# cvxgrp/pymde

Measured on AMD Instinct MI355X. Metric: edges/sec/iter (avg_distortion fwd+bwd), n=1M |E|=50M d=2, higher is better.
Workload: dtype f32; 1 GPU; BASELINE configs[3] / SURVEY 8d config 4a: n=1000000, |E|=50000000 uniform-random edges (out-degree 50), d=2, penalties.Log1p(1.5), weights in {1,2}; seeded on the device with torch.Generator(0) (the survey's recipe uses numpy default_rng(0): same distribution, another stream; --survey-seed builds that one); parallelism=single GPU, parameter_stream=codebook: 2 distinct weights ride in the packed half-edge word (4 B/half-edge)

## Files before the change

### pymde_amd/csrc/mde_ring_kernel.h

```cpp
#pragma once
#include <algorithm>
#include <cstring>
#include <type_traits>
#include <vector>

#include "mde_ring.h"
#define COMMA ,

#define MDE_RING23(FN, LIN)                                    \
  do {                                                         \
    FN fn{a};                                                  \
    int rc;                                                    \
    if (A.d == 2)                                              \
      rc = launch_ring<2, FN, LIN>(A, fn, nblocks);            \
    else                                                       \
      rc = launch_ring<3, FN, LIN>(A, fn, nblocks);            \
    return rc == MDE_OK ? 1 : rc;                              \
  } while (0)

typedef uint32_t ring_u4 __attribute__((ext_vector_type(4)));
typedef float ring_f4 __attribute__((ext_vector_type(4)));

template <int D>
struct RingVec;
template <>
struct RingVec<1> {
  typedef float T;
};
template <>
struct RingVec<2> {
  typedef float2 T;
};
template <>
struct RingVec<4> {
// ... 41 lines not shown
    q[0] = v[0];
    q[1] = v[1];
    q[2] = v[2];
  } else {
    typename RingVec<D>::T t;
    float* q = reinterpret_cast<float*>(&t);
#pragma unroll
    for (int c = 0; c < D; ++c) q[c] = v[c];
    *reinterpret_cast<typename RingVec<D>::T*>(p) = t;
  }
}

__device__ __forceinline__ void ring_ctrl_store(uint32_t addr, int v) {
  asm volatile("ds_write_b32 %0, %1" ::"v"(addr), "v"(v) : "memory");
}
__device__ __forceinline__ void ring_ctrl_store_counted(char* lds_base, uint32_t addr, int v) {
  typedef __attribute__((address_space(3))) volatile int* lds_vint;
  *(lds_vint)(lds_base + addr) = v;
}
__device__ __forceinline__ int ring_ctrl_load(uint32_t addr) {
  int v;
  asm volatile("ds_read_b32 %0, %1\n\ts_waitcnt lgkmcnt(0)" : "=&v"(v) : "v"(addr) : "memory");
  return v;
}

#if MDE_RING_ABLATE
static __device__ unsigned long long g_ring_probe[8][1024];
static __device__ int g_ring_diag[64][8];
static __device__ int g_ring_ndiag;
#ifndef MDE_RING_SPINMAX
#define MDE_RING_SPINMAX 100000
#endif
#define RING_CLK() __builtin_readcyclecounter()
#endif
#ifndef MDE_RING_FWORDS
#define MDE_RING_FWORDS 0
#endif
#ifdef MDE_RING_EVAL2
constexpr bool defined_MDE_RING_EVAL2 = true;
#else
constexpr bool defined_MDE_RING_EVAL2 = false;
#endif
template <int D, class Fn, bool HAS_GRAD, int PS, bool LIN>
__global__ __launch_bounds__(MDE_RING_BS) void k_fused_ring(
    int nloc, int row_lo, int n, int R, int Q, int NC, int ring_off, int S, const int32_t* __restrict__ wave_iter,
    const uint32_t* __restrict__ hdr, const uint32_t* __restrict__ packed, const uint32_t* __restrict__ bidx,
    const int32_t* __restrict__ slot_row, const float* __restrict__ a0, const float* __restrict__ a1, int a0_scalar, int a1_scalar,
    const float* __restrict__ X,
    float* __restrict__ grad, float* __restrict__ partial, double* __restrict__ loss_partials, Fn fn,
    float fix_value, float grad_scale, float* __restrict__ loss_out, double loss_scale, int fold, int dbg_arg) {
#if MDE_RING_ABLATE
#ifndef MDE_RING_ABLATE_MASK
#define MDE_RING_ABLATE_MASK (~0)
#endif
  const int dbg = dbg_arg & (MDE_RING_ABLATE_MASK);
#else
  constexpr int dbg = 0;
#endif
  constexpr int BS = MDE_RING_BS, NCW = MDE_RING_NCW, NPROD = MDE_RING_NPROD;
  constexpr bool CB = PS == 1, BX = PS == 2;
  constexpr int GR_OFF = ring_gr_off(D), CTRL_PROG = MDE_RING_CTRL_PROG(D), CTRL_F = MDE_RING_CTRL_F(D), CTRL_CB = MDE_RING_CTRL_CB(D);
  constexpr int C = ring_chunk_cols(D), CBYTES = ring_chunk_bytes(D), PIECES = CBYTES / 1024;
  static_assert(GR_OFF + (ring_row_cap(D) + 32) * 4 * D <= 65536 + GR_OFF && GR_OFF < 65536 && CTRL_CB + 32 < 65536,
                "region bases must fit the 16-bit offset of the LDS instructions");
  static_assert(NPROD <= 8 && NCW <= 16, "control-word layout");
  __shared__ __attribute__((aligned(16))) char L[MDE_RING_LDS_BYTES];
  float* XR = reinterpret_cast<float*>(L);
  float* GR = reinterpret_cast<float*>(L + GR_OFF);
  const int tid = threadIdx.x, lane = tid & 63;
  const int wave = __builtin_amdgcn_readfirstlane(tid >> 6);
  const int rb = blockIdx.x / Q, qg = blockIdx.x % Q;
  const int j_lo = (int)(((int64_t)qg * NC + Q - 1) / Q), j_hi = (int)(((int64_t)(qg + 1) * NC + Q - 1) / Q);
  const int r0 = rb * R;
  const int nr = min(R, nloc - r0);
  const uint32_t dummy_row = (uint32_t)R * 4u * (uint32_t)D;
  const float a0s = (a0_scalar && PS == 0) ? a0[0] : 1.0f;
  const uint32_t tab_off = (uint32_t)ring_off + (uint32_t)S * (uint32_t)CBYTES;
  const float a1s = (a1 && a1_scalar) ? a1[0] : 0.0f;
  const bool a1_arr = a1 && !a1_scalar;
  {
    float4* z = reinterpret_cast<float4*>(L + GR_OFF);
    const int nz = ((R + 32) * 4 * D + 15) / 16;
    for (int i = tid; i < nz; i += BS) z[i] = make_float4(0.f, 0.f, 0.f, 0.f);
    const float* Xrow = X + (size_t)(row_lo + r0) * D;
    if (slot_row) {
      const int32_t* sr = slot_row + (size_t)rb * R;
      for (int sl = tid; sl < R; sl += BS) {
        const int r = sr[sl];
        float xv[D];
#pragma unroll
        for (int c = 0; c < D; ++c) xv[c] = r >= 0 ? X[(size_t)(row_lo + r) * D + c] : 0.0f;
#pragma unroll
        for (int c = 0; c < D; ++c) XR[sl * D + c] = xv[c];
      }
    } else if ((reinterpret_cast<uintptr_t>(Xrow) & 15) == 0) {
      const ring_f4* X4 = reinterpret_cast<const ring_f4*>(Xrow);
      ring_f4* XR4 = reinterpret_cast<ring_f4*>(L);
      const int n4 = (nr * D) >> 2;
      for (int i0 = 0; i0 < n4; i0 += 8 * BS) {
        ring_f4 t[8];
#pragma unroll
        for (int k = 0; k < 8; ++k) t[k] = X4[min(i0 + tid + k * BS, max(n4 - 1, 0))];
#pragma unroll
        for (int k = 0; k < 8; ++k)
          if (i0 + tid + k * BS < n4) XR4[i0 + tid + k * BS] = t[k];
      }
      for (int i = (n4 << 2) + tid; i < nr * D; i += BS) XR[i] = Xrow[i];
    } else {
      for (int i = tid; i < nr * D; i += BS) XR[i] = Xrow[i];
    }
    if (tid < 32 * D) XR[R * D + tid] = 0.0f;
    int* prog = reinterpret_cast<int*>(L + CTRL_PROG);
    int* F = reinterpret_cast<int*>(L + CTRL_F);
    if (tid < 16) prog[tid] = (tid < NCW) ? j_lo : MDE_RING_DONE;
#if MDE_RING_FWORDS
    static_assert(NPROD == 4 && MDE_RING_UNIT == 1, "MDE_RING_FWORDS: four producers, one chunk per step");
    if (tid >= 16 && tid < 16 + NPROD) F[tid - 16] = (j_lo + (tid - 16) < j_hi) ? j_lo + (tid - 16) : MDE_RING_DONE;
#else
    if (tid == 16) F[0] = j_lo;
#endif
    if (CB && tid >= 32 && tid < 32 + MDE_RING_CB_VALUES)
      reinterpret_cast<float*>(L + CTRL_CB)[tid - 32] = a0[tid - 32] * Fn::kParamScale;
    if (BX && tid >= 64 && tid < 64 + MDE_RING_BX_VALUES)
      reinterpret_cast<float*>(L + tab_off)[tid - 64] = a0[tid - 64] * Fn::kParamScale;
  }
  __syncthreads();
  float loss = 0.0f, loss2 = 0.0f;

  if (wave >= NCW) {
    if (MDE_RING_PRODPRIO) __builtin_amdgcn_s_setprio(MDE_RING_PRODPRIO);
    const int p = wave - NCW;
    const char* Xb = reinterpret_cast<const char*>(X);
    const size_t nbytes = (size_t)n * D * 4;
    const size_t last16 = nbytes - 16;
    constexpr int DEPTH = MDE_RING_DEPTH, UNIT = MDE_RING_UNIT;
    ring_f4 buf[DEPTH][UNIT * PIECES];
    auto ld16 = [&](ring_f4& dst, const ring_f4* src) __attribute__((always_inline)) {
#if MDE_RING_ASMLOAD
      asm volatile("global_load_dwordx4 %0, %1, off" : "=v"(dst) : "v"(src) : "memory");
#else
      dst = *src;
#endif
    };
    auto fetch = [&](int k, int j0u) __attribute__((always_inline)) {
#pragma unroll
      for (int c = 0; c < UNIT; ++c) {
        const int j = j0u + c;
        if (j < NC - 1) {
          const ring_f4* src = reinterpret_cast<const ring_f4*>(Xb + (size_t)j * CBYTES + (size_t)lane * 16);
#pragma unroll
          for (int i = 0; i < PIECES; ++i) ld16(buf[k][c * PIECES + i], src + i * 64);
        } else {
          const size_t off0 = (size_t)min(j, NC - 1) * CBYTES + (size_t)lane * 16;
#pragma unroll
          for (int i = 0; i < PIECES; ++i) {
            const size_t off = off0 + (size_t)i * 1024;
            ld16(buf[k][c * PIECES + i], reinterpret_cast<const ring_f4*>(Xb + (off < last16 ? off : last16)));
          }
        }
// ... 8 lines not shown
      else if constexpr (UNIT * PIECES == 3)
        asm volatile("s_waitcnt vmcnt(%3)" : "+v"(buf[k][0]), "+v"(buf[k][1]), "+v"(buf[k][2]) : "n"(NEWER) : "memory");
      else if constexpr (UNIT * PIECES == 2)
        asm volatile("s_waitcnt vmcnt(%2)" : "+v"(buf[k][0]), "+v"(buf[k][1]) : "n"(NEWER) : "memory");
      else if constexpr (UNIT * PIECES == 6)
        asm volatile("s_waitcnt vmcnt(%6)" : "+v"(buf[k][0]), "+v"(buf[k][1]), "+v"(buf[k][2]), "+v"(buf[k][3]), "+v"(buf[k][4]),
                     "+v"(buf[k][5]) : "n"(NEWER) : "memory");
      else
        asm volatile("s_waitcnt vmcnt(%8)" : "+v"(buf[k][0]), "+v"(buf[k][1]), "+v"(buf[k][2]), "+v"(buf[k][3]), "+v"(buf[k][4]),
                     "+v"(buf[k][5]), "+v"(buf[k][6]), "+v"(buf[k][7]) : "n"(NEWER) : "memory");
#endif
    };
    ring_f4 tail_v = {0.0f, 0.0f, 0.0f, 0.0f};
    int tail_rel = -1;
    if ((nbytes & 15) != 0 && j_hi == NC) {
      const size_t off_str = nbytes & ~(size_t)15;
      const size_t rel = off_str - (size_t)(NC - 1) * CBYTES;
      if (off_str >= (size_t)(NC - 1) * CBYTES && lane == (int)((rel & 1023) >> 4)) {
        tail_rel = (int)rel;
        const float* tp = reinterpret_cast<const float*>(Xb + off_str);
        const int nt = (int)((nbytes - off_str) >> 2);
        tail_v[0] = tp[0];
        if (nt > 1) tail_v[1] = tp[1];
        if (nt > 2) tail_v[2] = tp[2];
      }
    }
    int minprog = j_lo, landed = j_lo;
    const uint32_t poll_addr = lane < 16 ? CTRL_PROG + 4u * (uint32_t)lane : (uint32_t)CTRL_F;
#if MDE_RING_ABLATE
    unsigned long long pr_t0 = RING_CLK(), pr_blocked = 0, pr_polls = 0, pr_chain = 0, pr_data = 0, pr_write = 0;
#endif
#pragma unroll
    for (int k = 0; k < DEPTH; ++k) fetch(k, j_lo + UNIT * (p + k * NPROD));
    int slot = (j_lo + UNIT * p) % S;
    for (int j0 = j_lo + UNIT * p; j0 < j_hi && !(dbg & 128); j0 += UNIT * DEPTH * NPROD) {
#pragma unroll
      for (int k = 0; k < DEPTH; ++k) {
        const int j = j0 + k * UNIT * NPROD;
        if (j < j_hi) {
          const int jl = min(j + UNIT, j_hi) - 1;
          while (jl - S >= minprog && !(dbg & 8)) {
#if MDE_RING_ABLATE
            const unsigned long long tb0 = RING_CLK();
            ++pr_polls;
#endif
            int v = ring_ctrl_load(poll_addr);
            asm volatile("s_nop 1\n\tv_min_i32_dpp %0, %0, %0 row_shr:1 row_mask:0xf bank_mask:0xf\n\t"
                         "s_nop 1\n\tv_min_i32_dpp %0, %0, %0 row_shr:2 row_mask:0xf bank_mask:0xf\n\t"
                         "s_nop 1\n\tv_min_i32_dpp %0, %0, %0 row_shr:4 row_mask:0xf bank_mask:0xf\n\ts_nop 1"
                         : "+v"(v));
            if (NCW > 8) asm volatile("v_min_i32_dpp %0, %0, %0 row_shr:8 row_mask:0xf bank_mask:0xf\n\ts_nop 1" : "+v"(v));
            minprog = __builtin_amdgcn_readlane(v, NCW <= 8 ? 7 : 15);
            landed = __builtin_amdgcn_readlane(v, 16);
            if (jl - S >= minprog) __builtin_amdgcn_s_sleep(MDE_RING_PSLEEP);
#if MDE_RING_ABLATE
            pr_blocked += RING_CLK() - tb0;
            if (pr_polls > MDE_RING_SPINMAX) {
              if (lane == 0) {
                const int kk = atomicAdd(&g_ring_ndiag, 1);
                if (kk < 64) {
                  int* r = g_ring_diag[kk];
                  r[0] = 2; r[1] = blockIdx.x; r[2] = p; r[3] = j; r[4] = minprog; r[5] = S; r[6] = j_lo; r[7] = j_hi;
                }
              }
              pr_polls = 0;
              minprog = jl;
// ... 15 lines not shown
            const int jc = j + c;
            if (UNIT > 1 && jc >= j_hi) break;
            int sc = slot + c;
            if (UNIT > 1 && sc >= S) sc -= S;
            char* dst = L + (uint32_t)__builtin_amdgcn_readfirstlane(ring_off + sc * CBYTES) + lane * 16;
#pragma unroll
            for (int i = 0; i < PIECES; ++i) *reinterpret_cast<ring_f4*>(dst + i * 1024) = buf[k][c * PIECES + i];
            if (jc == NC - 1 && tail_rel >= 0) *reinterpret_cast<ring_f4*>(dst - lane * 16 + tail_rel) = tail_v;
          }
          asm volatile("" ::: "memory");
#if MDE_RING_FWORDS
          (void)landed;
          ring_ctrl_store_counted(L, CTRL_F + 4u * (uint32_t)p, (j + NPROD < j_hi) ? j + NPROD : MDE_RING_DONE);
#else
          while (landed != j && !(dbg & 8)) {
            landed = __builtin_amdgcn_readfirstlane(ring_ctrl_load((uint32_t)CTRL_F + 0u * (uint32_t)lane));
#if MDE_RING_ABLATE
            ++pr_chain;
#endif
            if (landed != j) __builtin_amdgcn_s_sleep(0);
          }
          ring_ctrl_store_counted(L, CTRL_F, jl + 1);
#endif
#if MDE_RING_ABLATE
          if (dbg & 512) pr_write += RING_CLK() - td0;
#endif
          fetch(k, j + UNIT * DEPTH * NPROD);
          slot += UNIT * NPROD;
          while (slot >= S) slot -= S;
        }
      }
    }
#if MDE_RING_ABLATE
    if ((dbg & 512) && lane == 0 && blockIdx.x < 1024) {
      atomicAdd(&g_ring_probe[3][blockIdx.x], RING_CLK() - pr_t0);
      atomicAdd(&g_ring_probe[4][blockIdx.x], pr_blocked);
      atomicAdd(&g_ring_probe[6][blockIdx.x], pr_polls);
      atomicAdd(&g_ring_probe[5][blockIdx.x], pr_data);
      atomicAdd(&g_ring_probe[7][blockIdx.x], pr_write);
    }
#endif
  } else {
    if (MDE_RING_CONSPRIO) __builtin_amdgcn_s_setprio(MDE_RING_CONSPRIO);
    const int ib = __builtin_amdgcn_readfirstlane(wave_iter[blockIdx.x * NCW + wave]);
    const int NB = (__builtin_amdgcn_readfirstlane(wave_iter[blockIdx.x * NCW + wave + 1]) - ib) >> 2;
    if (NB > 0 && !(dbg & 64)) {
      const bool a0_arr = !a0_scalar && PS == 0;
      const uint32_t* bp = BX ? bidx + (size_t)(ib >> 2) * 64 + lane : nullptr;
      const ring_u4* sp = reinterpret_cast<const ring_u4*>(packed) + (size_t)(ib >> 2) * 64 + lane;
      const ring_f4* ap = reinterpret_cast<const ring_f4*>(a0_arr ? a0 : reinterpret_cast<const float*>(packed)) +
                          (size_t)(ib >> 2) * 64 + lane;
      const int lastb = NB - 1;
      constexpr int PFB = MDE_RING_PFB;
      ring_u4 pq[PFB] = {};
      uint32_t hv[PFB] = {};
      ring_f4 wq[PFB] = {};
      uint32_t bq[PFB] = {};
      const uint32_t* hvp = hdr + (size_t)ib * MDE_RING_HW + (lane & 15);
      auto load_block = [&](int u, int b) __attribute__((always_inline)) {
        const int bc = min(b, lastb);
#if defined(MDE_RING_STREAM_L2)
        pq[u] = sp[(size_t)(bc & 7) * 64];
#elif defined(MDE_RING_STREAM_NT)
        pq[u] = __builtin_nontemporal_load(&sp[(size_t)bc * 64]);
#else
        pq[u] = sp[(size_t)bc * 64];
#endif
        hv[u] = hvp[(size_t)bc * 16];
        if (PS == 0) wq[u] = ap[(size_t)bc * 64];
        if (BX) bq[u] = bp[(size_t)bc * 64];
      };
#if MDE_RING_ABLATE
      unsigned long long cs_t0 = RING_CLK(), cs_poll = 0, cs_trips = 0;
#endif

      struct Pre {
        float xr[D], xc[D], p0;
#ifdef MDE_RING_KEEPROW
        uint32_t row;
#endif
      };
#ifdef MDE_RING_PROBE_ROWLIN
      auto row_of = [&](uint32_t w) __attribute__((always_inline)) { return ((w & 0x7f00u) | ((uint32_t)lane << 3)) & 0xfff8u; };
#else
      auto row_of = [&](uint32_t w) __attribute__((always_inline)) { return D == 2 ? (w & 0xfff8u) : (w & 0xfffcu); };
#endif
#ifdef MDE_RING_PROBE_COLLIN
      auto col_of = [&](uint32_t w) __attribute__((always_inline)) {
        return (((w >> 13) & 0x3f000u) | ((uint32_t)lane << 3)) & 0x3fff8u;
      };
#else
      auto col_of = [&](uint32_t w) __attribute__((always_inline)) {
        return D == 2 ? ((w >> 13) & 0x3fff8u) : ((w >> 14) & 0x3fffcu);
      };
#endif
      auto issue_x = [&](uint32_t w, float p0, uint32_t bi4) __attribute__((always_inline)) {
        Pre r;
        if constexpr (BX)
          r.p0 = *reinterpret_cast<const float*>(L + tab_off + bi4);
        else
          r.p0 = CB ? *reinterpret_cast<const float*>(L + CTRL_CB + ((w & (D == 2 ? 7u : 3u)) << 2)) : p0 * Fn::kParamScale;
#ifdef MDE_RING_KEEPROW
        r.row = row_of(w);
        ring_ld_operand<D>(L, r.row, r.xr);
// ... 136 lines not shown

      Pre xa, xb;
      float acc[D], accb[D];
      auto block_body = [&](auto lc_tag, int u, int b) __attribute__((always_inline)) {
#pragma unroll
        for (int h = 0; h < 2; ++h) {
          const int q = 2 * h;
          const int un = h == 0 ? u : (u + 1) % PFB, qn = (q + 2) & 3;
          wait_pair(un, qn);
          const Pre xna = issue_x(pq[un][qn], (a0_scalar || PS != 0) ? a0s : wq[un][qn], bx4(bq[un], qn));
          const Pre xnb = issue_x(pq[un][qn + 1], (a0_scalar || PS != 0) ? a0s : wq[un][qn + 1], bx4(bq[un], qn + 1));
          release_to((u + 1) % PFB, q);
          prefetch_landed();
          const float p1a = a1_arr ? a1[((size_t)((ib >> 2) + b) * 64 + lane) * 4 + q] : a1s;
          const float p1b = a1_arr ? a1[((size_t)((ib >> 2) + b) * 64 + lane) * 4 + q + 1] : a1s;
          const bool lc2 = decltype(lc_tag)::value == 2;
          const uint32_t hma = lc2 ? (uint32_t)__builtin_amdgcn_readlane((int)hv[u], 4 * q) : 0u;
          const uint32_t hmb = lc2 ? (uint32_t)__builtin_amdgcn_readlane((int)hv[u], 4 * q + 4) : 0u;
          finish(lc_tag, pq[u][q], xa, acc, p1a, hma);
          if (HAS_GRAD) {
            const bool same = row_of(pq[u][q + 1]) == row_of(pq[u][q]);
#pragma unroll
            for (int c = 0; c < D; ++c) accb[c] = same ? acc[c] : accb[c];
          }
          finish(lc_tag, pq[u][q + 1], xb, accb, p1b, hmb);
          if (HAS_GRAD) {
            ring_ld<D>(L + GR_OFF + row_of(pq[un][qn]), acc);
            ring_ld<D>(L + GR_OFF + row_of(pq[un][qn + 1]), accb);
          }
          xa = xna;
          xb = xnb;
        }
      };
#pragma unroll
      for (int u = 0; u < PFB; ++u) load_block(u, u);
      release_to(0, 0);
      wait_pair(0, 0);
      xa = issue_x(pq[0][0], (a0_scalar || PS != 0) ? a0s : wq[0][0], bx4(bq[0], 0));
      xb = issue_x(pq[0][1], (a0_scalar || PS != 0) ? a0s : wq[0][1], bx4(bq[0], 1));
      release_to(0, 2);
      prefetch_landed();
      if (HAS_GRAD) {
        ring_ld<D>(L + GR_OFF + row_of(pq[0][0]), acc);
        ring_ld<D>(L + GR_OFF + row_of(pq[0][1]), accb);
      }
      for (int base = 0; base < NB; base += PFB) {
#pragma unroll
        for (int u = 0; u < PFB; ++u) {
          const int b = base + u;
          if (b < NB) {
            const int bcls = __builtin_amdgcn_readlane((int)hv[u], 3) & 3;
            if (bcls == 0)
              block_body(std::integral_constant<int, 0>(), u, b);
            else if (bcls == 1)
              block_body(std::integral_constant<int, 1>(), u, b);
            else
              block_body(std::integral_constant<int, 2>(), u, b);
          }
          load_block(u, b + PFB);
        }
      }
#if MDE_RING_ABLATE
      if ((dbg & 512) && lane == 0 && blockIdx.x < 1024) {
        atomicAdd(&g_ring_probe[0][blockIdx.x], RING_CLK() - cs_t0);
        atomicAdd(&g_ring_probe[1][blockIdx.x], cs_poll);
        atomicAdd(&g_ring_probe[2][blockIdx.x], cs_trips);
      }
#endif
    }
    if constexpr (Fn::kRingFused) loss = fmaf(loss, 0.6931471805599453f, loss2) * (1.0f / Fn::kParamScale);
    ring_ctrl_store_counted(L, CTRL_PROG + 4u * (uint32_t)wave, MDE_RING_DONE);
    __builtin_amdgcn_s_waitcnt(0x0F70);
  }
  __syncthreads();
  if (HAS_GRAD && slot_row) {
    const int32_t* sr = slot_row + (size_t)rb * R;
    if (fold) {
      unsigned int* sync = reinterpret_cast<unsigned int*>(partial + (size_t)Q * nloc * D) + 2 * rb;
      int* tk = reinterpret_cast<int*>(L + 512);
      if (tid == 0) *tk = (int)__hip_atomic_fetch_add(&sync[0], 1u, __ATOMIC_RELAXED, __HIP_MEMORY_SCOPE_AGENT);
      __syncthreads();
      const bool second = *tk != 0;
      float* mine = partial + (size_t)qg * nloc * D;
      const float* other = partial + (size_t)(1 - qg) * nloc * D;
      if (!second) {
        for (int sl = tid; sl < R; sl += BS) {
          const int r = sr[sl];
          if (r < 0) continue;
#pragma unroll
          for (int c = 0; c < D; ++c)
            __hip_atomic_store(mine + (size_t)r * D + c, GR[sl * D + c], __ATOMIC_RELAXED, __HIP_MEMORY_SCOPE_AGENT);
        }
        __builtin_amdgcn_s_waitcnt(0x0F70);
        __syncthreads();
        if (tid == 0) __hip_atomic_store(&sync[1], 1u, __ATOMIC_RELAXED, __HIP_MEMORY_SCOPE_AGENT);
      } else {
        if (tid == 0) {
          while (__hip_atomic_load(&sync[1], __ATOMIC_RELAXED, __HIP_MEMORY_SCOPE_AGENT) == 0u) __builtin_amdgcn_s_sleep(2);
          __hip_atomic_store(&sync[1], 0u, __ATOMIC_RELAXED, __HIP_MEMORY_SCOPE_AGENT);
          __hip_atomic_store(&sync[0], 0u, __ATOMIC_RELAXED, __HIP_MEMORY_SCOPE_AGENT);
        }
        __syncthreads();
        for (int s0 = 0; s0 < R; s0 += 8 * BS) {
          int rr[8];
          float o[8][D];
#pragma unroll
          for (int k = 0; k < 8; ++k) rr[k] = s0 + tid + k * BS < R ? sr[s0 + tid + k * BS] : -1;
#pragma unroll
          for (int k = 0; k < 8; ++k)
#pragma unroll
            for (int c = 0; c < D; ++c)
              o[k][c] = __hip_atomic_load(other + (size_t)max(rr[k], 0) * D + c, __ATOMIC_RELAXED, __HIP_MEMORY_SCOPE_AGENT);
#pragma unroll
          for (int k = 0; k < 8; ++k) {
            if (rr[k] < 0) continue;
            const int sl = s0 + tid + k * BS;
#pragma unroll
            for (int c = 0; c < D; ++c) {
              const float m = GR[sl * D + c];
              grad[(size_t)(row_lo + rr[k]) * D + c] = (qg == 0 ? m + o[k][c] : o[k][c] + m) * grad_scale;
            }
          }
        }
      }
      __syncthreads();
    } else {
      float* dst = (Q == 1) ? grad + (size_t)row_lo * D : partial + (size_t)qg * nloc * D;
      const float sc = (Q == 1) ? grad_scale : 1.0f;
      for (int sl = tid; sl < R; sl += BS) {
        const int r = sr[sl];
        if (r < 0) continue;
#pragma unroll
        for (int c = 0; c < D; ++c) dst[(size_t)r * D + c] = GR[sl * D + c] * sc;
      }
    }
  } else if (HAS_GRAD && fold) {
    unsigned int* sync = reinterpret_cast<unsigned int*>(partial + (size_t)Q * nloc * D) + 2 * rb;
    int* tk = reinterpret_cast<int*>(L + 512);
    if (tid == 0) *tk = (int)__hip_atomic_fetch_add(&sync[0], 1u, __ATOMIC_RELAXED, __HIP_MEMORY_SCOPE_AGENT);
    __syncthreads();
    const bool second = *tk != 0;
    float* mine = partial + ((size_t)qg * nloc + r0) * D;
    const float* other = partial + ((size_t)(1 - qg) * nloc + r0) * D;
    float* grow = grad + (size_t)(row_lo + r0) * D;
    static_assert(GR_OFF % 16 == 0, "16-byte accumulator pieces");
    const bool vec = ((reinterpret_cast<uintptr_t>(mine) | reinterpret_cast<uintptr_t>(other) | reinterpret_cast<uintptr_t>(grow)) & 15) == 0;
    const int n4 = vec ? (nr * D) >> 2 : 0, n1 = nr * D;
    const ring_f4* GR4 = reinterpret_cast<const ring_f4*>(GR);
    if (!second) {
      for (int i = tid; i < n4; i += BS) {
        const ring_f4 v4 = GR4[i];
        asm volatile("global_store_dwordx4 %0, %1, off sc1" ::"v"(reinterpret_cast<ring_f4*>(mine) + i), "v"(v4) : "memory");
      }
      for (int i = (n4 << 2) + tid; i < n1; i += BS) __hip_atomic_store(mine + i, GR[i], __ATOMIC_RELAXED, __HIP_MEMORY_SCOPE_AGENT);
      __builtin_amdgcn_s_waitcnt(0x0F70);
      __syncthreads();
      if (tid == 0) __hip_atomic_store(&sync[1], 1u, __ATOMIC_RELAXED, __HIP_MEMORY_SCOPE_AGENT);
    } else {
      if (tid == 0) {
        while (__hip_atomic_load(&sync[1], __ATOMIC_RELAXED, __HIP_MEMORY_SCOPE_AGENT) == 0u) __builtin_amdgcn_s_sleep(2);
        __hip_atomic_store(&sync[1], 0u, __ATOMIC_RELAXED, __HIP_MEMORY_SCOPE_AGENT);
        __hip_atomic_store(&sync[0], 0u, __ATOMIC_RELAXED, __HIP_MEMORY_SCOPE_AGENT);
      }
      __syncthreads();
      const ring_f4* o4p = reinterpret_cast<const ring_f4*>(other);
      for (int i0 = 0; i0 < n4; i0 += 8 * BS) {
        ring_f4 o[8];
#pragma unroll
        for (int k = 0; k < 8; ++k)
          asm volatile("global_load_dwordx4 %0, %1, off sc1" : "=v"(o[k]) : "v"(o4p + min(i0 + tid + k * BS, n4 - 1)) : "memory");
        asm volatile("s_waitcnt vmcnt(0)" : "+v"(o[0]), "+v"(o[1]), "+v"(o[2]), "+v"(o[3]), "+v"(o[4]), "+v"(o[5]), "+v"(o[6]), "+v"(o[7])::"memory");
#pragma unroll
        for (int k = 0; k < 8; ++k) {
          const int i = i0 + tid + k * BS;
          if (i < n4) {
            const ring_f4 m = GR4[i];
            reinterpret_cast<ring_f4*>(grow)[i] = (qg == 0 ? m + o[k] : o[k] + m) * grad_scale;
          }
        }
      }
      for (int i0 = n4 << 2; i0 < n1; i0 += 8 * BS) {
        float o[8];
#pragma unroll
        for (int k = 0; k < 8; ++k) o[k] = __hip_atomic_load(other + min(i0 + tid + k * BS, n1 - 1), __ATOMIC_RELAXED, __HIP_MEMORY_SCOPE_AGENT);
#pragma unroll
        for (int k = 0; k < 8; ++k) {
          const int i = i0 + tid + k * BS;
          if (i < n1) grow[i] = (qg == 0 ? GR[i] + o[k] : o[k] + GR[i]) * grad_scale;
        }
      }
    }
    __syncthreads();
  } else if (HAS_GRAD) {
    float* grow = (Q == 1) ? grad + (size_t)(row_lo + r0) * D : partial + ((size_t)qg * nloc + r0) * D;
    const float sc = (Q == 1) ? grad_scale : 1.0f;
    const int n4 = (reinterpret_cast<uintptr_t>(grow) & 15) == 0 ? (nr * D) >> 2 : 0;
    for (int i = tid; i < n4; i += BS) reinterpret_cast<ring_f4*>(grow)[i] = reinterpret_cast<const ring_f4*>(GR)[i] * sc;
    for (int i = (n4 << 2) + tid; i < nr * D; i += BS) grow[i] = GR[i] * sc;
  }
  double* red = reinterpret_cast<double*>(L);
  unsigned int* ticket = reinterpret_cast<unsigned int*>(loss_partials + MDE_MAX_PARTIALS);
  const double v = mde_wave_sum((double)loss);
  if (lane == 0) red[wave] = v;
  __syncthreads();
  if (tid == 0) {
    double s = 0.0;
    for (int i = 0; i < NCW; ++i) s += red[i];
    mde_st_partial(loss_partials + blockIdx.x, s);
  }
  int* last_flag = reinterpret_cast<int*>(L + 256);
  __builtin_amdgcn_s_waitcnt(0x0F70);
  __syncthreads();
  if (tid == 0) {
    const unsigned int k = __hip_atomic_fetch_add(ticket, 1u, __ATOMIC_RELAXED, __HIP_MEMORY_SCOPE_AGENT);
    *last_flag = (k == gridDim.x - 1u) ? 1 : 0;
    if (*last_flag) __hip_atomic_store(ticket, 0u, __ATOMIC_RELAXED, __HIP_MEMORY_SCOPE_AGENT);
  }
  __syncthreads();
  if (!*last_flag) return;
  double t = 0.0;
  for (int i = tid; i < (int)gridDim.x; i += BS) t += mde_ld_partial(loss_partials + i);
  t = mde_wave_sum(t);
  __syncthreads();
  if (lane == 0) red[wave] = t;
  __syncthreads();
  if (tid == 0) {
    double s = 0.0;
    for (int i = 0; i < BS / 64; ++i) s += red[i];
    *loss_out = (float)(s * loss_scale);
    loss_partials[MDE_PARTIALS_LOSS_D] = s * loss_scale;
  }
}

template <class V>
__global__ __launch_bounds__(MDE_BLOCK) void k_ring_combine(int64_t m, int Q, const V* __restrict__ partial,
                                                            float scale, V* __restrict__ out) {
  constexpr int W = sizeof(V) / sizeof(float);
  const int64_t i = (int64_t)blockIdx.x * MDE_BLOCK + threadIdx.x;
  if (i >= m) return;
  V a[8];
#pragma unroll
  for (int q = 0; q < 8; ++q)
    if (q < Q) a[q] = partial[(size_t)q * m + i];
  float s[W];
#pragma unroll
  for (int k = 0; k < W; ++k) s[k] = reinterpret_cast<const float*>(&a[0])[k];
#pragma unroll
  for (int q = 1; q < 8; ++q)
    if (q < Q) {
#pragma unroll
      for (int k = 0; k < W; ++k) s[k] += reinterpret_cast<const float*>(&a[q])[k];
// ... 38 lines not shown
  const uint32_t* bidx = bx ? reinterpret_cast<const uint32_t*>(A.a0) : nullptr;
  const float* a0 = cb ? A.a0 + L.H : (bx ? A.a0 + L.H / 4 : A.a0);
  const int Q = L.col_groups;
  *nblocks = L.n_row_blocks * Q;
  const float out_scale = A.grad_scale * A.inv_p;
  const float fix_value = A.inv_p > 0.0f ? 1.0f / A.inv_p : 1.0f;
#if MDE_RING_ABLATE
  const int dbg = getenv("MDE_RING_DBG") ? atoi(getenv("MDE_RING_DBG")) : 0;
#else
  const int dbg = 0;
#endif
  static const int fold_env = getenv("MDE_RING_FOLD") ? atoi(getenv("MDE_RING_FOLD")) : 1;
  const int fold = (Q == 2 && A.grad && fold_env) ? 1 : 0;
  hipLaunchKernelGGL(kern, dim3(L.n_row_blocks * Q), dim3(MDE_RING_BS), 0, A.st,
                     (int)(A.plan->row_hi - A.plan->row_lo), (int)A.plan->row_lo, (int)A.plan->n,
                     L.rows_per_block, Q, L.n_chunks, L.ring_off, L.slots, L.wave_iter, L.hdr, stream, bidx, L.slot_row, a0, A.a1,
                     A.a0_scalar, A.a1_scalar, A.X, A.grad, L.partial, A.plan->partials, fn, fix_value, out_scale,
                     A.loss_out, (L.count_all ? 1.0 : 2.0) * A.loss_scale, fold, dbg);
  MDE_LAUNCH_CHECK();
#if MDE_RING_ABLATE
  {
    static int dl = 0;
    if (++dl == 3) {
      int nd = 0;
      int hd[64][8];
      (void)hipStreamSynchronize(A.st);
      (void)hipMemcpyFromSymbol(&nd, HIP_SYMBOL(g_ring_ndiag), sizeof(int));
      (void)hipMemcpyFromSymbol(hd, HIP_SYMBOL(g_ring_diag), sizeof(hd));
      fprintf(stderr, "[mde ring diag] %d give-ups in the first launches\n", nd);
      for (int k = 0; k < nd && k < 24; ++k)
        fprintf(stderr, hd[k][0] == 1 ? "[mde ring diag] consumer wg %d wave %d: need %d ready %d m %d slot %d NB %d\n"
                                      : "[mde ring diag] producer wg %d p %d: j %d minprog %d infl %d oldest %d j_hi %d\n",
                hd[k][1], hd[k][2], hd[k][3], hd[k][4], hd[k][5], hd[k][6], hd[k][7]);
    }
  }
  if (dbg & 512) {
    static int launches = 0;
    if (++launches == 8) {
      std::vector<unsigned long long> h(8 * 1024);
      (void)hipStreamSynchronize(A.st);
      (void)hipMemcpyFromSymbol(h.data(), HIP_SYMBOL(g_ring_probe), sizeof(unsigned long long) * 8 * 1024);
      const int nb = std::min(1024, L.n_row_blocks * Q);
      double s[8] = {0};
      for (int k = 0; k < 8; ++k)
        for (int i = 0; i < nb; ++i) s[k] += (double)h[k * 1024 + i];
      const double L8 = 8.0 * nb;
      fprintf(stderr, "[mde ring probe] per consumer wave and launch: loop %.0f clk, in chunk polls %.0f clk (%.1f%%), %.0f poll trips | "
              "per producer wave: loop %.0f clk, blocked on a slot %.0f (%.1f%%), waiting for the chunk's loads %.0f (%.1f%%), %.0f slot polls, LDS stores + ordered publish %.0f clk\n",
              s[0] / L8 / MDE_RING_NCW, s[1] / L8 / MDE_RING_NCW, 100.0 * s[1] / s[0], s[2] / L8 / MDE_RING_NCW,
              s[3] / L8 / MDE_RING_NPROD, s[4] / L8 / MDE_RING_NPROD, 100.0 * s[4] / s[3], s[5] / L8 / MDE_RING_NPROD,
              100.0 * s[5] / s[3], s[6] / L8 / MDE_RING_NPROD, s[7] / L8 / MDE_RING_NPROD);
      std::vector<double> loop(nb), work(nb);
      for (int i = 0; i < nb; ++i) {
        loop[i] = (double)h[i] / 8.0 / MDE_RING_NCW;
        work[i] = ((double)h[i] - (double)h[1024 + i]) / 8.0 / MDE_RING_NCW;
      }
      auto quant = [&](std::vector<double> v, const char* what) {
        std::sort(v.begin(), v.end());
        double m = 0;
        for (double x : v) m += x;
        fprintf(stderr, "[mde ring probe] per workgroup, %s: min %.0f p10 %.0f median %.0f mean %.0f p90 %.0f max %.0f clk\n", what, v[0],
                v[v.size() / 10], v[v.size() / 2], m / v.size(), v[v.size() * 9 / 10], v.back());
      };
      quant(loop, "consumer loop");
      quant(work, "consumer loop minus polls");
      for (int q8 = 0; q8 < 8; ++q8) {
// ... 28 lines not shown
```

Before: 319.0 billion edges/s/iter.

## Split ring kernel prologue by role and symmetrize the cross-block gradient fold

The prologue no longer uses a whole-block __syncthreads before the producer/consumer split. Producers issue their first global fetches, then zero the LDS accumulators and control words. Consumers load X rows and prefetch their first edge blocks before a lightweight s_barrier, so the setup overlaps the initial memory latency. The two-block gradient fold is made symmetric: each block publishes the half the other needs, meets through a flag handshake, then finalizes its own half, instead of one block writing everything and the other waiting to do all the combining. The loss ticket is merged into that meeting point, and timestamp instrumentation is added under the ablation build flag. The risk is subtle synchronization and LDS-ordering bugs from the raw barrier and the mutual spin-wait.

```diff
diff --git a/pymde_amd/csrc/mde_ring_kernel.h b/pymde_amd/csrc/mde_ring_kernel.h
--- a/pymde_amd/csrc/mde_ring_kernel.h
+++ b/pymde_amd/csrc/mde_ring_kernel.h
@@ -1,5 +1,6 @@
 #pragma once
 #include <algorithm>
+#include <cstdio>
 #include <cstring>
 #include <type_traits>
 #include <vector>
@@ -107,6 +108,11 @@
 #define MDE_RING_SPINMAX 100000
 #endif
 #define RING_CLK() __builtin_readcyclecounter()
+#define MDE_RING_NSTAMP 32
+static __device__ unsigned long long g_ring_stamp[1024][MDE_RING_NSTAMP];
+#define RING_STAMP(var) var = RING_CLK()
+#else
+#define RING_STAMP(var) (void)0
 #endif
 #ifndef MDE_RING_FWORDS
 #define MDE_RING_FWORDS 0
@@ -131,6 +137,12 @@
   const int dbg = dbg_arg & (MDE_RING_ABLATE_MASK);
 #else
   constexpr int dbg = 0;
+#endif
+#if MDE_RING_ABLATE
+  unsigned long long ts_entry = RING_CLK(), ts_pro = 0, ts_fold = 0, ts_raised = 0, ts_seen = 0, ts_done = 0;
+  auto put_stamp = [&](int k, unsigned long long t) __attribute__((always_inline)) {
+    if ((dbg & 4096) && blockIdx.x < 1024) g_ring_stamp[blockIdx.x][k] = t;
+  };
 #endif
   constexpr int BS = MDE_RING_BS, NCW = MDE_RING_NCW, NPROD = MDE_RING_NPROD;
   constexpr bool CB = PS == 1, BX = PS == 2;
@@ -153,14 +165,34 @@
   const uint32_t tab_off = (uint32_t)ring_off + (uint32_t)S * (uint32_t)CBYTES;
   const float a1s = (a1 && a1_scalar) ? a1[0] : 0.0f;
   const bool a1_arr = a1 && !a1_scalar;
-  {
+  constexpr int CT = NCW * 64, PT = NPROD * 64;
+  auto prologue_barrier = [&]() __attribute__((always_inline)) { asm volatile("s_waitcnt lgkmcnt(0)\n\ts_barrier" ::: "memory"); };
+  auto prologue_lds = [&](int pt) __attribute__((always_inline)) {
     float4* z = reinterpret_cast<float4*>(L + GR_OFF);
     const int nz = ((R + 32) * 4 * D + 15) / 16;
-    for (int i = tid; i < nz; i += BS) z[i] = make_float4(0.f, 0.f, 0.f, 0.f);
+    for (int i = pt; i < nz; i += PT) z[i] = make_float4(0.f, 0.f, 0.f, 0.f);
+    static_assert(32 * D <= PT && 16 + NPROD <= PT, "one prologue word per producer thread");
+    if (pt < 32 * D) XR[R * D + pt] = 0.0f;
+    int* prog = reinterpret_cast<int*>(L + CTRL_PROG);
+    int* F = reinterpret_cast<int*>(L + CTRL_F);
+    if (pt < 16) prog[pt] = (pt < NCW) ? j_lo : MDE_RING_DONE;
+#if MDE_RING_FWORDS
+    static_assert(NPROD == 4 && MDE_RING_UNIT == 1, "MDE_RING_FWORDS: four producers, one chunk per step");
+    if (pt >= 16 && pt < 16 + NPROD) F[pt - 16] = (j_lo + (pt - 16) < j_hi) ? j_lo + (pt - 16) : MDE_RING_DONE;
+#else
+    if (pt == 16) F[0] = j_lo;
+#endif
+  };
+  auto prologue_rows = [&](int ct, auto&& between) __attribute__((always_inline)) {
+    static_assert(32 + MDE_RING_CB_VALUES <= CT && 64 + MDE_RING_BX_VALUES <= CT, "the tables' threads are consumer threads");
+    const bool cb_t = CB && ct >= 32 && ct < 32 + MDE_RING_CB_VALUES, bx_t = BX && ct >= 64 && ct < 64 + MDE_RING_BX_VALUES;
+    float tabv = 0.0f;
+    if (cb_t) tabv = a0[ct - 32] * Fn::kParamScale;
+    if (bx_t) tabv = a0[ct - 64] * Fn::kParamScale;
     const float* Xrow = X + (size_t)(row_lo + r0) * D;
     if (slot_row) {
       const int32_t* sr = slot_row + (size_t)rb * R;
-      for (int sl = tid; sl < R; sl += BS) {
+      for (int sl = ct; sl < R; sl += CT) {
         const int r = sr[sl];
         float xv[D];
 #pragma unroll
@@ -168,38 +200,42 @@
 #pragma unroll
         for (int c = 0; c < D; ++c) XR[sl * D + c] = xv[c];
       }
+      between();
     } else if ((reinterpret_cast<uintptr_t>(Xrow) & 15) == 0) {
       const ring_f4* X4 = reinterpret_cast<const ring_f4*>(Xrow);
       ring_f4* XR4 = reinterpret_cast<ring_f4*>(L);
       const int n4 = (nr * D) >> 2;
-      for (int i0 = 0; i0 < n4; i0 += 8 * BS) {
-        ring_f4 t[8];
-#pragma unroll
-        for (int k = 0; k < 8; ++k) t[k] = X4[min(i0 + tid + k * BS, max(n4 - 1, 0))];
+      ring_f4 t[8];
+      auto ldb = [&](int i0) __attribute__((always_inline)) {
+#pragma unroll
+        for (int k = 0; k < 8; ++k) t[k] = X4[min(i0 + ct + k * CT, n4 - 1)];
+      };
+      auto stb = [&](int i0) __attribute__((always_inline)) {
 #pragma unroll
         for (int k = 0; k < 8; ++k)
-          if (i0 + tid + k * BS < n4) XR4[i0 + tid + k * BS] = t[k];
-      }
-      for (int i = (n4 << 2) + tid; i < nr * D; i += BS) XR[i] = Xrow[i];
+          if (i0 + ct + k * CT < n4) XR4[i0 + ct + k * CT] = t[k];
+      };
+      if (n4 > 0) {
+        ldb(0);
+        asm volatile("" ::: "memory");
+        between();
+        asm volatile("" ::: "memory");
+        stb(0);
+        for (int i0 = 8 * CT; i0 < n4; i0 += 8 * CT) {
+          ldb(i0);
+          stb(i0);
+        }
+      } else {
+        between();
+      }
+      for (int i = (n4 << 2) + ct; i < nr * D; i += CT) XR[i] = Xrow[i];
     } else {
-      for (int i = tid; i < nr * D; i += BS) XR[i] = Xrow[i];
-    }
-    if (tid < 32 * D) XR[R * D + tid] = 0.0f;
-    int* prog = reinterpret_cast<int*>(L + CTRL_PROG);
-    int* F = reinterpret_cast<int*>(L + CTRL_F);
-    if (tid < 16) prog[tid] = (tid < NCW) ? j_lo : MDE_RING_DONE;
-#if MDE_RING_FWORDS
-    static_assert(NPROD == 4 && MDE_RING_UNIT == 1, "MDE_RING_FWORDS: four producers, one chunk per step");
-    if (tid >= 16 && tid < 16 + NPROD) F[tid - 16] = (j_lo + (tid - 16) < j_hi) ? j_lo + (tid - 16) : MDE_RING_DONE;
-#else
-    if (tid == 16) F[0] = j_lo;
-#endif
-    if (CB && tid >= 32 && tid < 32 + MDE_RING_CB_VALUES)
-      reinterpret_cast<float*>(L + CTRL_CB)[tid - 32] = a0[tid - 32] * Fn::kParamScale;
-    if (BX && tid >= 64 && tid < 64 + MDE_RING_BX_VALUES)
-      reinterpret_cast<float*>(L + tab_off)[tid - 64] = a0[tid - 64] * Fn::kParamScale;
-  }
-  __syncthreads();
+      for (int i = ct; i < nr * D; i += CT) XR[i] = Xrow[i];
+      between();
+    }
+    if (cb_t) reinterpret_cast<float*>(L + CTRL_CB)[ct - 32] = tabv;
+    if (bx_t) reinterpret_cast<float*>(L + tab_off)[ct - 64] = tabv;
+  };
   float loss = 0.0f, loss2 = 0.0f;
 
   if (wave >= NCW) {
@@ -274,6 +310,9 @@
 #endif
 #pragma unroll
     for (int k = 0; k < DEPTH; ++k) fetch(k, j_lo + UNIT * (p + k * NPROD));
+    prologue_lds(tid - CT);
+    prologue_barrier();
+    RING_STAMP(ts_pro);
     int slot = (j_lo + UNIT * p) % S;
     for (int j0 = j_lo + UNIT * p; j0 < j_hi && !(dbg & 128); j0 += UNIT * DEPTH * NPROD) {
 #pragma unroll
@@ -355,6 +394,7 @@
       }
     }
 #if MDE_RING_ABLATE
+    if (lane == 0) put_stamp(18 + p, RING_CLK());
     if ((dbg & 512) && lane == 0 && blockIdx.x < 1024) {
       atomicAdd(&g_ring_probe[3][blockIdx.x], RING_CLK() - pr_t0);
       atomicAdd(&g_ring_probe[4][blockIdx.x], pr_blocked);
@@ -393,6 +433,12 @@
         if (PS == 0) wq[u] = ap[(size_t)bc * 64];
         if (BX) bq[u] = bp[(size_t)bc * 64];
       };
+      prologue_rows(tid, [&]() __attribute__((always_inline)) {
+#pragma unroll
+        for (int u = 0; u < PFB; ++u) load_block(u, u);
+      });
+      prologue_barrier();
+      RING_STAMP(ts_pro);
 #if MDE_RING_ABLATE
       unsigned long long cs_t0 = RING_CLK(), cs_poll = 0, cs_trips = 0;
 #endif
@@ -595,8 +641,6 @@
           xb = xnb;
         }
       };
-#pragma unroll
-      for (int u = 0; u < PFB; ++u) load_block(u, u);
       release_to(0, 0);
       wait_pair(0, 0);
       xa = issue_x(pq[0][0], (a0_scalar || PS != 0) ? a0s : wq[0][0], bx4(bq[0], 0));
@@ -607,6 +651,9 @@
         ring_ld<D>(L + GR_OFF + row_of(pq[0][0]), acc);
         ring_ld<D>(L + GR_OFF + row_of(pq[0][1]), accb);
       }
+#if MDE_RING_ABLATE
+      cs_t0 = RING_CLK();
+#endif
       for (int base = 0; base < NB; base += PFB) {
 #pragma unroll
         for (int u = 0; u < PFB; ++u) {
@@ -624,162 +671,164 @@
         }
       }
 #if MDE_RING_ABLATE
+      if (lane == 0) {
+        put_stamp(2 + wave, cs_t0);
+        put_stamp(10 + wave, RING_CLK());
+      }
       if ((dbg & 512) && lane == 0 && blockIdx.x < 1024) {
         atomicAdd(&g_ring_probe[0][blockIdx.x], RING_CLK() - cs_t0);
         atomicAdd(&g_ring_probe[1][blockIdx.x], cs_poll);
         atomicAdd(&g_ring_probe[2][blockIdx.x], cs_trips);
       }
 #endif
+    } else {
+      prologue_rows(tid, []() {});
+      prologue_barrier();
+      RING_STAMP(ts_pro);
     }
     if constexpr (Fn::kRingFused) loss = fmaf(loss, 0.6931471805599453f, loss2) * (1.0f / Fn::kParamScale);
     ring_ctrl_store_counted(L, CTRL_PROG + 4u * (uint32_t)wave, MDE_RING_DONE);
     __builtin_amdgcn_s_waitcnt(0x0F70);
   }
+  const double wave_loss = mde_wave_sum((double)loss);
   __syncthreads();
-  if (HAS_GRAD && slot_row) {
+  RING_STAMP(ts_fold);
+  double* red = reinterpret_cast<double*>(L);
+  int* last_flag = reinterpret_cast<int*>(L + 256);
+  unsigned int* ticket = reinterpret_cast<unsigned int*>(loss_partials + MDE_MAX_PARTIALS);
+  if (lane == 0) red[wave] = wave_loss;
+  auto loss_ticket = [&]() __attribute__((always_inline)) {
+    double s = 0.0;
+    for (int i = 0; i < NCW; ++i) s += red[i];
+    mde_st_partial(loss_partials + blockIdx.x, s);
+    __builtin_amdgcn_s_waitcnt(0x0F70);
+    const unsigned int k = __hip_atomic_fetch_add(ticket, 1u, __ATOMIC_RELAXED, __HIP_MEMORY_SCOPE_AGENT);
+    *last_flag = (k == gridDim.x - 1u) ? 1 : 0;
+    if (k == gridDim.x - 1u) __hip_atomic_store(ticket, 0u, __ATOMIC_RELAXED, __HIP_MEMORY_SCOPE_AGENT);
+  };
+  constexpr int LT = 64;
+  auto fold_meet = [&](unsigned int* sync) __attribute__((always_inline)) {
+    __builtin_amdgcn_s_waitcnt(0x0F70);
+    __syncthreads();
+    if (tid == 0) {
+      __hip_atomic_store(&sync[qg], 1u, __ATOMIC_RELAXED, __HIP_MEMORY_SCOPE_AGENT);
+      RING_STAMP(ts_raised);
+      while (__hip_atomic_load(&sync[1 - qg], __ATOMIC_RELAXED, __HIP_MEMORY_SCOPE_AGENT) == 0u) __builtin_amdgcn_s_sleep(2);
+      __hip_atomic_store(&sync[1 - qg], 0u, __ATOMIC_RELAXED, __HIP_MEMORY_SCOPE_AGENT);
+      RING_STAMP(ts_seen);
+    }
+    if (tid == LT) loss_ticket();
+    __syncthreads();
+  };
+  if (HAS_GRAD && fold && slot_row) {
     const int32_t* sr = slot_row + (size_t)rb * R;
-    if (fold) {
-      unsigned int* sync = reinterpret_cast<unsigned int*>(partial + (size_t)Q * nloc * D) + 2 * rb;
-      int* tk = reinterpret_cast<int*>(L + 512);
-      if (tid == 0) *tk = (int)__hip_atomic_fetch_add(&sync[0], 1u, __ATOMIC_RELAXED, __HIP_MEMORY_SCOPE_AGENT);
-      __syncthreads();
-      const bool second = *tk != 0;
-      float* mine = partial + (size_t)qg * nloc * D;
-      const float* other = partial + (size_t)(1 - qg) * nloc * D;
-      if (!second) {
-        for (int sl = tid; sl < R; sl += BS) {
-          const int r = sr[sl];
-          if (r < 0) continue;
-#pragma unroll
-          for (int c = 0; c < D; ++c)
-            __hip_atomic_store(mine + (size_t)r * D + c, GR[sl * D + c], __ATOMIC_RELAXED, __HIP_MEMORY_SCOPE_AGENT);
-        }
-        __builtin_amdgcn_s_waitcnt(0x0F70);
-        __syncthreads();
-        if (tid == 0) __hip_atomic_store(&sync[1], 1u, __ATOMIC_RELAXED, __HIP_MEMORY_SCOPE_AGENT);
-      } else {
-        if (tid == 0) {
-          while (__hip_atomic_load(&sync[1], __ATOMIC_RELAXED, __HIP_MEMORY_SCOPE_AGENT) == 0u) __builtin_amdgcn_s_sleep(2);
-          __hip_atomic_store(&sync[1], 0u, __ATOMIC_RELAXED, __HIP_MEMORY_SCOPE_AGENT);
-          __hip_atomic_store(&sync[0], 0u, __ATOMIC_RELAXED, __HIP_MEMORY_SCOPE_AGENT);
-        }
-        __syncthreads();
-        for (int s0 = 0; s0 < R; s0 += 8 * BS) {
-          int rr[8];
-          float o[8][D];
-#pragma unroll
-          for (int k = 0; k < 8; ++k) rr[k] = s0 + tid + k * BS < R ? sr[s0 + tid + k * BS] : -1;
-#pragma unroll
-          for (int k = 0; k < 8; ++k)
-#pragma unroll
-            for (int c = 0; c < D; ++c)
-              o[k][c] = __hip_atomic_load(other + (size_t)max(rr[k], 0) * D + c, __ATOMIC_RELAXED, __HIP_MEMORY_SCOPE_AGENT);
-#pragma unroll
-          for (int k = 0; k < 8; ++k) {
-            if (rr[k] < 0) continue;
-            const int sl = s0 + tid + k * BS;
-#pragma unroll
-            for (int c = 0; c < D; ++c) {
-              const float m = GR[sl * D + c];
-              grad[(size_t)(row_lo + rr[k]) * D + c] = (qg == 0 ? m + o[k][c] : o[k][c] + m) * grad_scale;
-            }
-          }
-        }
-      }
-      __syncthreads();
-    } else {
-      float* dst = (Q == 1) ? grad + (size_t)row_lo * D : partial + (size_t)qg * nloc * D;
-      const float sc = (Q == 1) ? grad_scale : 1.0f;
-      for (int sl = tid; sl < R; sl += BS) {
-        const int r = sr[sl];
-        if (r < 0) continue;
-#pragma unroll
-        for (int c = 0; c < D; ++c) dst[(size_t)r * D + c] = GR[sl * D + c] * sc;
+    unsigned int* sync = reinterpret_cast<unsigned int*>(partial + (size_t)Q * nloc * D) + 2 * rb;
+    float* mine = partial + (size_t)qg * nloc * D;
+    const float* other = partial + (size_t)(1 - qg) * nloc * D;
+    const int sh = R >> 1;
+    const int my_lo = qg == 0 ? 0 : sh, my_hi = qg == 0 ? sh : R, ot_lo = qg == 0 ? sh : 0, ot_hi = qg == 0 ? R : sh;
+    for (int sl = ot_lo + tid; sl < ot_hi; sl += BS) {
+      const int r = sr[sl];
+      if (r < 0) continue;
+#pragma unroll
+      for (int c = 0; c < D; ++c)
+        __hip_atomic_store(mine + (size_t)r * D + c, GR[sl * D + c], __ATOMIC_RELAXED, __HIP_MEMORY_SCOPE_AGENT);
+    }
+    fold_meet(sync);
+    for (int s0 = my_lo; s0 < my_hi; s0 += 8 * BS) {
+      int rr[8];
+      float o[8][D];
+#pragma unroll
+      for (int k = 0; k < 8; ++k) rr[k] = s0 + tid + k * BS < my_hi ? sr[s0 + tid + k * BS] : -1;
+#pragma unroll
+      for (int k = 0; k < 8; ++k)
+#pragma unroll
+        for (int c = 0; c < D; ++c)
+          o[k][c] = __hip_atomic_load(other + (size_t)max(rr[k], 0) * D + c, __ATOMIC_RELAXED, __HIP_MEMORY_SCOPE_AGENT);
+#pragma unroll
+      for (int k = 0; k < 8; ++k) {
+        if (rr[k] < 0) continue;
+        const int sl = s0 + tid + k * BS;
+#pragma unroll
+        for (int c = 0; c < D; ++c) {
+          const float m = GR[sl * D + c];
+          grad[(size_t)(row_lo + rr[k]) * D + c] = (qg == 0 ? m + o[k][c] : o[k][c] + m) * grad_scale;
+        }
       }
     }
   } else if (HAS_GRAD && fold) {
     unsigned int* sync = reinterpret_cast<unsigned int*>(partial + (size_t)Q * nloc * D) + 2 * rb;
-    int* tk = reinterpret_cast<int*>(L + 512);
-    if (tid == 0) *tk = (int)__hip_atomic_fetch_add(&sync[0], 1u, __ATOMIC_RELAXED, __HIP_MEMORY_SCOPE_AGENT);
-    __syncthreads();
-    const bool second = *tk != 0;
     float* mine = partial + ((size_t)qg * nloc + r0) * D;
     const float* other = partial + ((size_t)(1 - qg) * nloc + r0) * D;
     float* grow = grad + (size_t)(row_lo + r0) * D;
     static_assert(GR_OFF % 16 == 0, "16-byte accumulator pieces");
     const bool vec = ((reinterpret_cast<uintptr_t>(mine) | reinterpret_cast<uintptr_t>(other) | reinterpret_cast<uintptr_t>(grow)) & 15) == 0;
     const int n4 = vec ? (nr * D) >> 2 : 0, n1 = nr * D;
+    const int s4 = n4 >> 1, se = vec ? s4 << 2 : n1 >> 1;
+    const int my_p_lo = qg == 0 ? 0 : s4, my_p_hi = qg == 0 ? s4 : n4, ot_p_lo = qg == 0 ? s4 : 0, ot_p_hi = qg == 0 ? n4 : s4;
+    const int my_l_lo = qg == 0 ? (vec ? se : 0) : (vec ? n4 << 2 : se), my_l_hi = qg == 0 ? se : n1;
+    const int ot_l_lo = qg == 0 ? (vec ? n4 << 2 : se) : (vec ? se : 0), ot_l_hi = qg == 0 ? n1 : se;
     const ring_f4* GR4 = reinterpret_cast<const ring_f4*>(GR);
-    if (!second) {
-      for (int i = tid; i < n4; i += BS) {
-        const ring_f4 v4 = GR4[i];
-        asm volatile("global_store_dwordx4 %0, %1, off sc1" ::"v"(reinterpret_cast<ring_f4*>(mine) + i), "v"(v4) : "memory");
-      }
-      for (int i = (n4 << 2) + tid; i < n1; i += BS) __hip_atomic_store(mine + i, GR[i], __ATOMIC_RELAXED, __HIP_MEMORY_SCOPE_AGENT);
-      __builtin_amdgcn_s_waitcnt(0x0F70);
-      __syncthreads();
-      if (tid == 0) __hip_atomic_store(&sync[1], 1u, __ATOMIC_RELAXED, __HIP_MEMORY_SCOPE_AGENT);
-    } else {
-      if (tid == 0) {
-        while (__hip_atomic_load(&sync[1], __ATOMIC_RELAXED, __HIP_MEMORY_SCOPE_AGENT) == 0u) __builtin_amdgcn_s_sleep(2);
-        __hip_atomic_store(&sync[1], 0u, __ATOMIC_RELAXED, __HIP_MEMORY_SCOPE_AGENT);
-        __hip_atomic_store(&sync[0], 0u, __ATOMIC_RELAXED, __HIP_MEMORY_SCOPE_AGENT);
-      }
-      __syncthreads();
-      const ring_f4* o4p = reinterpret_cast<const ring_f4*>(other);
-      for (int i0 = 0; i0 < n4; i0 += 8 * BS) {
-        ring_f4 o[8];
-#pragma unroll
-        for (int k = 0; k < 8; ++k)
-          asm volatile("global_load_dwordx4 %0, %1, off sc1" : "=v"(o[k]) : "v"(o4p + min(i0 + tid + k * BS, n4 - 1)) : "memory");
-        asm volatile("s_waitcnt vmcnt(0)" : "+v"(o[0]), "+v"(o[1]), "+v"(o[2]), "+v"(o[3]), "+v"(o[4]), "+v"(o[5]), "+v"(o[6]), "+v"(o[7])::"memory");
-#pragma unroll
-        for (int k = 0; k < 8; ++k) {
-          const int i = i0 + tid + k * BS;
-          if (i < n4) {
-            const ring_f4 m = GR4[i];
-            reinterpret_cast<ring_f4*>(grow)[i] = (qg == 0 ? m + o[k] : o[k] + m) * grad_scale;
-          }
-        }
-      }
-      for (int i0 = n4 << 2; i0 < n1; i0 += 8 * BS) {
-        float o[8];
-#pragma unroll
-        for (int k = 0; k < 8; ++k) o[k] = __hip_atomic_load(other + min(i0 + tid + k * BS, n1 - 1), __ATOMIC_RELAXED, __HIP_MEMORY_SCOPE_AGENT);
-#pragma unroll
-        for (int k = 0; k < 8; ++k) {
-          const int i = i0 + tid + k * BS;
-          if (i < n1) grow[i] = (qg == 0 ? GR[i] + o[k] : o[k] + GR[i]) * grad_scale;
-        }
-      }
+    for (int i = ot_p_lo + tid; i < ot_p_hi; i += BS) {
+      const ring_f4 v4 = GR4[i];
+      asm volatile("global_store_dwordx4 %0, %1, off sc1" ::"v"(reinterpret_cast<ring_f4*>(mine) + i), "v"(v4) : "memory");
+    }
+    for (int i = ot_l_lo + tid; i < ot_l_hi; i += BS) __hip_atomic_store(mine + i, GR[i], __ATOMIC_RELAXED, __HIP_MEMORY_SCOPE_AGENT);
+    fold_meet(sync);
+    const ring_f4* o4p = reinterpret_cast<const ring_f4*>(other);
+    for (int i0 = my_p_lo; i0 < my_p_hi; i0 += 8 * BS) {
+      ring_f4 o[8];
+#pragma unroll
+      for (int k = 0; k < 8; ++k)
+        asm volatile("global_load_dwordx4 %0, %1, off sc1" : "=v"(o[k]) : "v"(o4p + min(i0 + tid + k * BS, my_p_hi - 1)) : "memory");
+      asm volatile("s_waitcnt vmcnt(0)" : "+v"(o[0]), "+v"(o[1]), "+v"(o[2]), "+v"(o[3]), "+v"(o[4]), "+v"(o[5]), "+v"(o[6]), "+v"(o[7])::"memory");
+#pragma unroll
+      for (int k = 0; k < 8; ++k) {
+        const int i = i0 + tid + k * BS;
+        if (i < my_p_hi) {
+          const ring_f4 m = GR4[i];
+          reinterpret_cast<ring_f4*>(grow)[i] = (qg == 0 ? m + o[k] : o[k] + m) * grad_scale;
+        }
+      }
+    }
+    for (int i0 = my_l_lo; i0 < my_l_hi; i0 += 8 * BS) {
+      float o[8];
+#pragma unroll
+      for (int k = 0; k < 8; ++k) o[k] = __hip_atomic_load(other + min(i0 + tid + k * BS, my_l_hi - 1), __ATOMIC_RELAXED, __HIP_MEMORY_SCOPE_AGENT);
+#pragma unroll
+      for (int k = 0; k < 8; ++k) {
+        const int i = i0 + tid + k * BS;
+        if (i < my_l_hi) grow[i] = (qg == 0 ? GR[i] + o[k] : o[k] + GR[i]) * grad_scale;
+      }
+    }
+  } else {
+    if (HAS_GRAD && slot_row) {
+      const int32_t* sr = slot_row + (size_t)rb * R;
+      float* dst = (Q == 1) ? grad + (size_t)row_lo * D : partial + (size_t)qg * nloc * D;
+      const float sc = (Q == 1) ? grad_scale : 1.0f;
+      for (int sl = tid; sl < R; sl += BS) {
+        const int r = sr[sl];
+        if (r < 0) continue;
+#pragma unroll
+        for (int c = 0; c < D; ++c) dst[(size_t)r * D + c] = GR[sl * D + c] * sc;
+      }
+    } else if (HAS_GRAD) {
+      float* grow = (Q == 1) ? grad + (size_t)(row_lo + r0) * D : partial + ((size_t)qg * nloc + r0) * D;
+      const float sc = (Q == 1) ? grad_scale : 1.0f;
+      const int n4 = (reinterpret_cast<uintptr_t>(grow) & 15) == 0 ? (nr * D) >> 2 : 0;
+      for (int i = tid; i < n4; i += BS) reinterpret_cast<ring_f4*>(grow)[i] = reinterpret_cast<const ring_f4*>(GR)[i] * sc;
+      for (int i = (n4 << 2) + tid; i < nr * D; i += BS) grow[i] = GR[i] * sc;
     }
     __syncthreads();
-  } else if (HAS_GRAD) {
-    float* grow = (Q == 1) ? grad + (size_t)(row_lo + r0) * D : partial + ((size_t)qg * nloc + r0) * D;
-    const float sc = (Q == 1) ? grad_scale : 1.0f;
-    const int n4 = (reinterpret_cast<uintptr_t>(grow) & 15) == 0 ? (nr * D) >> 2 : 0;
-    for (int i = tid; i < n4; i += BS) reinterpret_cast<ring_f4*>(grow)[i] = reinterpret_cast<const ring_f4*>(GR)[i] * sc;
-    for (int i = (n4 << 2) + tid; i < nr * D; i += BS) grow[i] = GR[i] * sc;
-  }
-  double* red = reinterpret_cast<double*>(L);
-  unsigned int* ticket = reinterpret_cast<unsigned int*>(loss_partials + MDE_MAX_PARTIALS);
-  const double v = mde_wave_sum((double)loss);
-  if (lane == 0) red[wave] = v;
-  __syncthreads();
+    if (tid == 0) loss_ticket();
+    __syncthreads();
+  }
+#if MDE_RING_ABLATE
   if (tid == 0) {
-    double s = 0.0;
-    for (int i = 0; i < NCW; ++i) s += red[i];
-    mde_st_partial(loss_partials + blockIdx.x, s);
-  }
-  int* last_flag = reinterpret_cast<int*>(L + 256);
-  __builtin_amdgcn_s_waitcnt(0x0F70);
-  __syncthreads();
-  if (tid == 0) {
-    const unsigned int k = __hip_atomic_fetch_add(ticket, 1u, __ATOMIC_RELAXED, __HIP_MEMORY_SCOPE_AGENT);
-    *last_flag = (k == gridDim.x - 1u) ? 1 : 0;
-    if (*last_flag) __hip_atomic_store(ticket, 0u, __ATOMIC_RELAXED, __HIP_MEMORY_SCOPE_AGENT);
-  }
-  __syncthreads();
+    put_stamp(0, ts_entry); put_stamp(1, ts_pro); put_stamp(22, ts_fold); put_stamp(23, ts_raised);
+    put_stamp(24, ts_seen); put_stamp(25, RING_CLK()); put_stamp(26, RING_CLK());
+  }
+#endif
   if (!*last_flag) return;
   double t = 0.0;
   for (int i = tid; i < (int)gridDim.x; i += BS) t += mde_ld_partial(loss_partials + i);
@@ -884,6 +933,24 @@
         fprintf(stderr, hd[k][0] == 1 ? "[mde ring diag] consumer wg %d wave %d: need %d ready %d m %d slot %d NB %d\n"
                                       : "[mde ring diag] producer wg %d p %d: j %d minprog %d infl %d oldest %d j_hi %d\n",
                 hd[k][1], hd[k][2], hd[k][3], hd[k][4], hd[k][5], hd[k][6], hd[k][7]);
+    }
+  }
+  if (dbg & 4096) {
+    static int stamped = 0;
+    const char* path = getenv("MDE_RING_STAMPS");
+    const int at = getenv("MDE_RING_STAMPS_LAUNCH") ? atoi(getenv("MDE_RING_STAMPS_LAUNCH")) : 8;
+    if (path && ++stamped == at) {
+      std::vector<unsigned long long> h((size_t)1024 * MDE_RING_NSTAMP);
+      (void)hipStreamSynchronize(A.st);
+      (void)hipMemcpyFromSymbol(h.data(), HIP_SYMBOL(g_ring_stamp), sizeof(unsigned long long) * h.size());
+      if (FILE* f = fopen(path, "w")) {
+        const int nb = std::min(1024, L.n_row_blocks * Q);
+        for (int i = 0; i < nb; ++i) {
+          for (int k = 0; k < MDE_RING_NSTAMP; ++k) fprintf(f, "%llu ", h[(size_t)i * MDE_RING_NSTAMP + k]);
+          fprintf(f, "\n");
+        }
+        fclose(f);
+      }
     }
   }
   if (dbg & 512) {
```

Measured after the change: 318.8 billion edges/s/iter (median of 2 runs). About the same (-0.1%).
